# AlexFuster/Neural_network_image_compression

Hardware: AMD Instinct MI355X
Metric: Megapixels/sec encode+decode (higher is better)
Workload: dtype fp32 (split-f16x3 MFMA); 1 GPU; config2: 64x256x256x3 u8 synthetic per GPU, encode+decode (torch seed 1000+rank); global_batch=64, parallelism=dp1, weights=seeded spread init (random-init weights of the architecture)

## Files before the change

neural_network_image_compression_amd/csrc/nic_kernels.h:

```cpp
#pragma once
#include <hip/hip_runtime.h>
#include <stdint.h>

#include <vector>

namespace nic {

int set_error(int code, const char* msg);

enum InMode { IN_F32 = 0, IN_U8_LATENT = 1, IN_SPLIT = 2, IN_SPLIT_DMA = 3, IN_U8_CODES = 4 };
enum OutMode { OUT_F32 = 0, OUT_U8_LATENT = 1, OUT_SPLIT = 2 };

enum LayerId {
  L_CONV1 = 0, L_CONV2, L_CONV3, L_CONV4, L_CONV8,
  L_DCONV1, L_DCONV5, L_DCONV6, L_DCONV7, L_DCONV8,
  L_COUNT
};

constexpr float kF16Limit = 65504.0f;
struct RangeGuard {
  int* flag = nullptr;
  const int* gate = nullptr;
  int* trips = nullptr;
  int epoch = 0;
};

struct ConvArgs {
  RangeGuard rg;
  const float* in;
  const uint8_t* in_u8;
  float* out;
  const float* res;
  const uint16_t* in_s;
  uint16_t* out_s;
  const uint16_t* res_s;
  const char* zero16;
  uint8_t* out_u8;
  float* out_f32_latent;
  const float* w;
  const uint16_t* wx;
  float wscale[2];
  const float* bias;
  int P, nimg;
  int H, W;
  int OH, OW;
  int pad_y, pad_x;
  int tiles_x;
  int tiles_y, ntiles;
  int ws_taps;
  int ws_ngrp;
  int ws_blk[9];
  int ws_xcd;
  uint32_t* hist_part;
  const uint16_t* wx2;
  float wscale2[2];
  const float* bias2;
  int seg_rows;
  const uint8_t* rgb;
  const uint16_t* wx1;
  float wscale1[2];
  const float* bias1;
  int H0, W0;
  int p1y, p1x;
  uint16_t* cplane;
  int cp_h, cp_w;
  float* proj;
  const uint16_t* proj_w;
  float proj_scale[2];
};

struct Conv1Args {
  RangeGuard rg;
  const uint8_t* rgb;
  float* out;
  uint16_t* out_s;
// ... 159 lines not shown
```

neural_network_image_compression_amd/csrc/nic_kernels.hip:

```cpp

#include <hip/hip_runtime.h>
#include <stdint.h>
#include <stdlib.h>
#include <string.h>

#include <algorithm>
#include <type_traits>
#include <utility>

#include "nic_kernels.h"


namespace nic {

static int device_cus();

typedef float f32x2 __attribute__((ext_vector_type(2)));
typedef float f32x4 __attribute__((ext_vector_type(4)));
template <class F, int... I>
__device__ __forceinline__ void static_for_impl(F&& f, std::integer_sequence<int, I...>) {
  (f(std::integral_constant<int, I>{}), ...);
}
template <int N, class F>
__device__ __forceinline__ void static_for(F&& f) {
// ... 433 lines not shown
                                        int gx0, int c, int pw) const {
#pragma unroll
    for (int i = 0; i < NPP; ++i) {
      const int piece = pw + i * NPW;
      if (NPP * NPW > NPIECE && piece >= NPIECE) break;
      int e = code[i];
      if constexpr (OPAQUE) asm volatile("" : "+v"(e));
      const int gy = gy0 + (e & 255), gx = gx0 + ((e >> 8) & 255);
      const bool ok = (e >> 24) && (unsigned)gy < (unsigned)H && (unsigned)gx < (unsigned)W;
      const size_t off = ((size_t)(unsigned)(gy * W + gx) * CIN + (size_t)(((e >> 16) & 255) + c * HS) * 4) * 4;
      dma16(ok ? base + off : zero16, buf + piece * 1024);
    }
  }
};

constexpr unsigned kDmaOOR = 0x80000000u;
constexpr int kBufWord3 = 0x00020000;
#ifdef NIC_DIAG_KTIME
__device__ unsigned long long g_ktime[16][2];
#define KT_BEGIN(sl)                                                                         \
  do {                                                                                       \
    if ((threadIdx.x & 63) == 0) atomicMin(&g_ktime[sl][0], __builtin_amdgcn_s_memrealtime()); \
  } while (0)
#define KT_END(sl)                                                                           \
  do {                                                                                       \
    if ((threadIdx.x & 63) == 0) atomicMax(&g_ktime[sl][1], __builtin_amdgcn_s_memrealtime()); \
  } while (0)
struct KtGuard {
  int sl;
  __device__ explicit KtGuard(int s) : sl(s) { KT_BEGIN(s); }
  __device__ ~KtGuard() { KT_END(sl); }
};
#define KT_SCOPE(sl) KtGuard kt_guard_(sl)
extern "C" int nic_diag_ktime(unsigned long long* out, int reset) {
  if (out && hipMemcpyFromSymbol(out, HIP_SYMBOL(g_ktime), sizeof(g_ktime)) != hipSuccess) return -1;
  if (reset) {
    unsigned long long init[16][2];
    for (int k = 0; k < 16; ++k) init[k][0] = ~0ull, init[k][1] = 0;
    if (hipMemcpyToSymbol(HIP_SYMBOL(g_ktime), init, sizeof(init)) != hipSuccess) return -1;
  }
  return hipDeviceSynchronize() == hipSuccess ? 0 : -1;
}
#else
#define KT_BEGIN(sl) do { } while (0)
#define KT_END(sl) do { } while (0)
#define KT_SCOPE(sl) do { } while (0)
#endif

__device__ __forceinline__ void dma16_buf(__amdgpu_buffer_rsrc_t rsrc, unsigned voff, char* lds_wave_base) {
  __builtin_amdgcn_raw_ptr_buffer_load_lds(rsrc, (lds_ptr_t)lds_wave_base, 16, (int)voff, 0, 0, 0);
}

template <class G, int CIN, int NPW>
struct HaloDma {
  static_assert(G::HW <= 15, "halo column packed into the low 4 bits of a 16-B aligned offset");
  static constexpr int PSS = G::PSB / 16, RPS = G::RPB / 16;
  static constexpr int TOTAL = G::HH * RPS;
  static constexpr int NPIECE = (TOTAL + 63) / 64;
  static constexpr int NPP = (NPIECE + NPW - 1) / NPW;
  unsigned off[NPP];
  __device__ __forceinline__ void init(int pw, int lane, int W) {
#pragma unroll
// ... 90 lines not shown
    }
    pl += d_pl;
  }
};

template <int CIN, int TH, int TW>
struct GeomWS {
  static_assert(CIN == 64, "record geometry searched for Cin 64");
  static constexpr int HH = TH + 2, HW = TW + 2;
  static constexpr bool S2 = false, SWZ = true;
  static constexpr int HE = HW;
  static constexpr int PSB = CIN * 4;
  static constexpr int RPB = HW * PSB;
  static constexpr int HALO_BYTES = HH * RPB;
  static_assert(HALO_BYTES % 1024 == 0, "whole DMA pieces");
  static __device__ __forceinline__ int chunk_at(int slot, int hx) { return slot ^ ((2 * hx) & 15); }
};

#ifndef NIC_RES_DMA
#define NIC_RES_DMA 1
#endif
constexpr bool kResDma = NIC_RES_DMA != 0;
template <int CIN, int COUT, int TH, int TW, bool RESID, int KH, int KW, bool TRP, bool PROJ = false>
__device__ __forceinline__ void ws_body(const ConvArgs& a, char* lds, int model, int bi, int nb, int tb, int py,
                                        int px, bool copy_w8 = true) {
  constexpr int NTAPS = KH * KW, NW = COUT / 16, KST = CIN / 32, MT = TH * TW / 16;
  static_assert(TW == 8 && CIN % 32 == 0 && COUT % 16 == 0, "16-pixel tiles = two 8-pixel rows");
  static_assert(!(TRP && RESID), "no residual on the transposed phases");
  static_assert(!PROJ || (TRP && COUT == 64 && TH * TW == 64), "projection: dconv7 8x8 tiles");
  using G = GeomWS<CIN, TH, TW>;
  constexpr bool kBufHalo = !RESID || kResDma;
  using HP = std::conditional_t<kBufHalo, HaloDma<G, CIN, NW>, HaloPieces<G, CIN, CIN, NW>>;
  constexpr int TAP_BYTES = CIN * COUT * 4;

  const int wave = __builtin_amdgcn_readfirstlane(threadIdx.x >> 6);
  const int lane = threadIdx.x & 63, g = lane >> 4, l16 = lane & 15;
  const int co0 = wave * 16 + 4 * g;
  const int per_plane = a.tiles_y * a.tiles_x;
  const int p0 = model ? a.nimg : 0, np = model ? a.P - a.nimg : a.nimg;
  const int ntot = np * per_plane;
  const int ntile = bi < ntot ? (ntot - bi + nb - 1) / nb : 0;

  f16x8 wr[NTAPS][KST][2];
  {
    const char* wsrc = (const char*)a.wx + ((size_t)model * a.ws_taps + tb) * TAP_BYTES;
#pragma unroll
    for (int t = 0; t < NTAPS; ++t)
#pragma unroll
      for (int ks = 0; ks < KST; ++ks)
#pragma unroll
        for (int hl = 0; hl < 2; ++hl)
          wr[t][ks][hl] = *(const f16x8*)(wsrc + (size_t)t * TAP_BYTES +
                                          ((((2 * ks + (g >> 1)) * 2 + hl) * 2 + (g & 1)) * COUT + wave * 16 + l16) * 16);
  }
  const float scale = a.wscale[model];
  const f32x4 bias = *(const f32x4*)(a.bias + model * COUT + co0);
  constexpr int W8F = 2 * KST * 2;
  const f16x8* w8lds = (const f16x8*)(lds + 2 * G::HALO_BYTES) + lane;
  const float scale8 = PROJ ? a.proj_scale[model] : 0.f;
  char* hproj = lds + 2 * G::HALO_BYTES + W8F * 64 * 16;
  if constexpr (PROJ)
    if (copy_w8) {
      const f16x8* src = (const f16x8*)a.proj_w + (size_t)model * W8F * 64;
      for (int q = threadIdx.x; q < W8F * 64; q += 64 * NW) ((f16x8*)(lds + 2 * G::HALO_BYTES))[q] = src[q];
    }

  int bx[KW];
#pragma unroll
  for (int kw = 0; kw < KW; ++kw) {
    const int hx = (l16 & 7) + kw;
    bx[kw] = (l16 >> 3) * G::RPB + hx * G::PSB + (G::chunk_at(g, hx) << 4);
  }

  HP hp;
  const unsigned plane_bytes = (unsigned)((size_t)a.H * a.W * CIN * 4);
  if constexpr (kBufHalo)
    hp.init(wave, lane, a.W);
  else
    hp.init(wave, lane);
  TileWalk it_issue, it_ep;
  it_issue.init(bi, nb, a.tiles_y, a.tiles_x);
  it_ep = it_issue;
  auto tile_take = [&](TileWalk& w, int& p, int& t0y, int& t0x) {
    int pl, ty, tx;
    w.take(pl, ty, tx);
    p = p0 + pl;
    t0y = ty * TH;
    t0x = tx * TW;
  };
  auto issue = [&](int i) {
    int p, t0y, t0x;
    tile_take(it_issue, p, t0y, t0x);
#ifdef NIC_DIAG_ONETILE
    p = p0;
    t0y = TH;
    t0x = TW;
#endif
    if constexpr (kBufHalo)
      hp.issue(lds + (i & 1) * G::HALO_BYTES, (const char*)a.in_s + (size_t)p * plane_bytes, plane_bytes, a.W,
               t0y - a.pad_y, t0x - a.pad_x, wave);
    else
      hp.template issue<true>(lds + (i & 1) * G::HALO_BYTES, (const char*)a.in_s + (size_t)p * plane_bytes, a.zero16,
                              a.H, a.W, t0y - a.pad_y, t0x - a.pad_x, 0, wave);
  };
// ... 199 lines not shown
#endif
}

template <int CIN, int TH, int TW>
struct GeomS2 {
  static constexpr int HH = (TH - 1) * 2 + 5, HW = (TW - 1) * 2 + 5, HE = (HW + 1) / 2;
  static constexpr int PSS = CIN / 4 + 2, PSB = PSS * 16;
  static constexpr int RPS = (HW * PSS + 7) / 8 * 8, RPB = RPS * 16;
  static constexpr int HTOT = HH * RPS;
  static constexpr int NPIECE = (HTOT + 63) / 64;
  static constexpr int HALO_BYTES = NPIECE * 1024;
  static __device__ __forceinline__ int col(int hx) { return (hx & 1) * HE + (hx >> 1); }
};


constexpr int C12_PH = 41;

#ifndef NIC_WS2_PRIO
#define NIC_WS2_PRIO 1
#endif
constexpr int HIST_R = 2;
constexpr int HIST_LDS = 2 * 256 * HIST_R * 4 + 2 * 2 * 2 * 64 * 4;
template <int CIN, int COUT, int NTS, int TH, int OUT_MODE, int TS, bool HIST = false>
__device__ __forceinline__ void ws2_wave(const ConvArgs& a, char* lds, int model, int bi, int nb) {
  constexpr int TW = 8, MT = TH * TW / 16, NCG = COUT / 16, KST = CIN / 32, NW = NCG * NTS;
  static_assert(!HIST || OUT_MODE == OUT_U8_LATENT, "histogram fold: conv8 only");
  constexpr int T0 = 25 * TS / NTS, T1 = 25 * (TS + 1) / NTS, NT = T1 - T0;
  using G = GeomS2<CIN, TH, TW>;
  constexpr int TAP_BYTES = CIN * COUT * 4;
  constexpr int NPP = (G::NPIECE + NW - 1) / NW;
  constexpr int PART = MT * 1024;
  char* part = lds + 2 * G::HALO_BYTES;

  const int wave = __builtin_amdgcn_readfirstlane(threadIdx.x >> 6);
  const int cg = wave % NCG;
  const int lane = threadIdx.x & 63, g = lane >> 4, l16 = lane & 15;
  const int per_plane = a.tiles_y * a.tiles_x;
  const int p0 = model ? a.nimg : 0, np = model ? a.P - a.nimg : a.nimg;
  const int ntot = np * per_plane;
  const int ntile = bi < ntot ? (ntot - bi + nb - 1) / nb : 0;
  uint32_t* hist = (uint32_t*)(part + 2 * (NTS - 1) * NCG * PART);
  uint32_t* codes = hist + 2 * 256 * HIST_R;
  int hcur = 0, hpend = -1;
  uint32_t hz = 0;
  int h1_p = 0, h1_y = 0, h1_x = 0, h2_p = 0, h2_y = 0, h2_x = 0;
  auto hist_flush = [&](int q) __attribute__((always_inline)) {
    uint32_t* hb = hist + (q & 1) * (256 * HIST_R);
    const int t = cg * 64 + lane;
#pragma unroll
    for (int h = 0; h < 2; ++h) {
      const int bin = t + 128 * h;
      uint32_t c = 0;
#pragma unroll
      for (int r = 0; r < HIST_R; ++r) {
        c += hb[bin * HIST_R + r];
        hb[bin * HIST_R + r] = 0;
      }
      if (c) atomicAdd(a.hist_part + (size_t)(p0 + q) * 256 + bin, c);
    }
  };
  auto hist_close = [&] __attribute__((always_inline)) {
    uint32_t z = hz;
    for (int o = 32; o > 0; o >>= 1) z += __shfl_xor(z, o);
// ... 24 lines not shown
      }
    }
  };

  f16x8 wr[NT][KST][2];
  {
    const char* wsrc = (const char*)a.wx + ((size_t)model * 25 + T0) * TAP_BYTES;
#pragma unroll
    for (int t = 0; t < NT; ++t)
#pragma unroll
      for (int ks = 0; ks < KST; ++ks)
#pragma unroll
        for (int hl = 0; hl < 2; ++hl)
          wr[t][ks][hl] = *(const f16x8*)(wsrc + (size_t)t * TAP_BYTES +
                                          ((((2 * ks + (g >> 1)) * 2 + hl) * 2 + (g & 1)) * COUT + cg * 16 + l16) * 16);
  }
  const float scale = a.wscale[model];
  const int co0 = cg * 16 + 4 * g;
  const f32x4 bias = *(const f32x4*)(a.bias + model * COUT + co0);
  int boff[MT];
#pragma unroll
  for (int m = 0; m < MT; ++m) boff[m] = 2 * (2 * m + (l16 >> 3)) * G::RPB + (l16 & 7) * G::PSB + g * 16;
  TileWalk w_issue, w_ep;
  w_issue.init(bi, nb, a.tiles_y, a.tiles_x);
  w_ep = w_issue;
  if constexpr (HIST)
    for (int q = threadIdx.x; q < 2 * 256 * HIST_R; q += 64 * NW) hist[q] = 0;
  auto tile_take = [&](TileWalk& w, int& p, int& t0y, int& t0x) {
    int pl, ty, tx;
    w.take(pl, ty, tx);
    p = p0 + pl;
    t0y = ty * TH;
    t0x = tx * TW;
  };
  unsigned doff[NPP];
  int drc[NPP];
#pragma unroll
  for (int j = 0; j < NPP; ++j) {
    const int piece = wave + j * NW;
    const int q = piece * 64 + lane;
    const int row = q / G::RPS, r = q - row * G::RPS;
    const int sp = r / G::PSS, k = r - sp * G::PSS;
    const int hx = sp < G::HE ? 2 * sp : 2 * (sp - G::HE) + 1;
    const bool ok = piece < G::NPIECE && q < G::HTOT && sp < G::HW && k < CIN / 4;
    doff[j] = ok ? (unsigned)((row * a.W + hx) * CIN * 4 + k * 16) : kDmaOOR;
    drc[j] = row << 8 | hx;
  }
// ... 257 lines not shown
  }
#pragma unroll
  for (int k = 0; k < 3; ++k) {
    unsigned hw[2], lw[2];
#pragma unroll
    for (int h = 0; h < 2; ++h) {
      const _Float16 h0 = (_Float16)v[k][2 * h], h1 = (_Float16)v[k][2 * h + 1];
      const _Float16 l0 = (_Float16)(v[k][2 * h] - (float)h0), l1 = (_Float16)(v[k][2 * h + 1] - (float)h1);
      hw[h] = (unsigned)__builtin_bit_cast(uint16_t, h0) | (unsigned)__builtin_bit_cast(uint16_t, h1) << 16;
      lw[h] = (unsigned)__builtin_bit_cast(uint16_t, l0) | (unsigned)__builtin_bit_cast(uint16_t, l1) << 16;
    }
    const size_t o = ((size_t)k * N + n) * plane + (size_t)yp * wp + 4 * q4;
    typedef unsigned int u32x2v __attribute__((ext_vector_type(2)));
    __builtin_nontemporal_store((u32x2v){hw[0], hw[1]}, (u32x2v*)(cp + o));
    __builtin_nontemporal_store((u32x2v){lw[0], lw[1]}, (u32x2v*)(cp + P * plane + o));
  }
}


#ifndef NIC_C12_REUSE
#define NIC_C12_REUSE 1
#endif
template <int ROLE>
__device__ __forceinline__ void c12r_wave(const ConvArgs& a, char* lds, int model, int bi, int nb) {
  constexpr int CIN = 32, COUT = 64, MT = 4, NCG = 4;
  using G = GeomS2<CIN, 8, 8>;
  constexpr int TAP_BYTES = CIN * COUT * 4;
  constexpr int PART = MT * 1024;
  char* accs = lds + 2 * G::HALO_BYTES;
  char* patches = accs + NCG * PART;
  int* pflag = (int*)(patches + 4 * C12_PLANE);
  const int wave = __builtin_amdgcn_readfirstlane(threadIdx.x >> 6);
  const int cg = wave & 3;
  const int lane = threadIdx.x & 63, g = lane >> 4, l16 = lane & 15;
  const int per_plane = a.tiles_y * a.tiles_x;
  const int p0 = model ? a.nimg : 0, np = model ? a.P - a.nimg : a.nimg;
  const int ntot = np * per_plane;
  constexpr bool CONTIG = NIC_C12_REUSE != 0;
  const int t_first = CONTIG ? (int)((long long)bi * ntot / nb) : bi;
  const int ntile = CONTIG ? (int)((long long)(bi + 1) * ntot / nb) - t_first : bi < ntot ? (ntot - bi + nb - 1) / nb : 0;
  const int t_step = CONTIG ? 1 : nb;
  float rmax = 0.f;
  if (threadIdx.x < NCG) pflag[threadIdx.x] = 0;
#ifdef NIC_STAMPS
  unsigned long long sx[8] = {}, sa, sb;
  const unsigned long long s_rt0 = __builtin_amdgcn_s_memrealtime(), s_c0 = __builtin_amdgcn_s_memtime();
  NIC_PNOW(sa);
#define C12R_MARK(kk)  \
  do {                 \
    NIC_PNOW(sb);      \
    sx[kk] += sb - sa; \
    sa = sb;           \
  } while (0)
#else
#define C12R_MARK(kk) \
  do {                \
  } while (0)
#endif

  if constexpr (ROLE == 2) {
    f16x8 wr[25][2];
    {
      const char* wsrc = (const char*)a.wx + (size_t)model * 25 * TAP_BYTES;
#pragma unroll
// ... 228 lines not shown
    }
  }
#ifdef NIC_STAMPS
  if (lane == 0) {
    unsigned long long* o = g_stamps + ((size_t)blockIdx.x * 8 + wave) * 8;
#pragma unroll
    for (int q = 0; q < 7; ++q) o[q] = sx[q];
    o[7] = ntile;
    if (wave == 0) {
      g_stamps[256 * 64 + 2 * blockIdx.x] = __builtin_amdgcn_s_memtime() - s_c0;
      g_stamps[256 * 64 + 2 * blockIdx.x + 1] = __builtin_amdgcn_s_memrealtime() - s_rt0;
    }
  }
#endif
#undef C12R_MARK
  range_report(a.rg, rmax);
}

__device__ __forceinline__ int xcd_pos(int b, int nb) {
  const int x = b & 7, q = nb >> 3, r = nb & 7;
  return x * q + (x < r ? x : r) + (b >> 3);
}

__global__ __launch_bounds__(512) void conv12_kernel(ConvArgs a) {
  KT_SCOPE(1);
  using G = GeomS2<32, 8, 8>;
  __shared__ __attribute__((aligned(16)))
  char lds[2 * G::HALO_BYTES + 4 * 4 * 1024 + 4 * C12_PLANE + 16];
  int gi = 0;
  while (gi + 1 < a.ws_ngrp && (int)blockIdx.x >= a.ws_blk[gi + 1]) ++gi;
  const int nb = a.ws_blk[gi + 1] - a.ws_blk[gi];
  const int bi = xcd_pos(blockIdx.x - a.ws_blk[gi], nb);
  if (__builtin_amdgcn_readfirstlane((int)(threadIdx.x >> 6)) < 4)
    c12r_wave<2>(a, lds, gi, bi, nb);
  else
    c12r_wave<1>(a, lds, gi, bi, nb);
}

template <int CIN, int COUT, int NTS, int TH, int OUT_MODE, bool HIST = false>
__global__ __launch_bounds__(64 * (COUT / 16) * NTS) void conv_ws2_kernel(ConvArgs a) {
  KT_SCOPE(3);
  using G = GeomS2<CIN, TH, 8>;
  constexpr int NCG = COUT / 16;
  static_assert(NCG * NTS == 8, "8 waves per block");
  constexpr int PARTS = 2 * (NTS - 1) * NCG * (TH / 2) * 1024;
  __shared__ __attribute__((aligned(16)))
  char lds[2 * G::HALO_BYTES + PARTS + (HIST ? HIST_LDS : 0)];
  int gi = 0;
  while (gi + 1 < a.ws_ngrp && (int)blockIdx.x >= a.ws_blk[gi + 1]) ++gi;
  const int nb = a.ws_blk[gi + 1] - a.ws_blk[gi];
  const int bi = xcd_pos(blockIdx.x - a.ws_blk[gi], nb);
  const int ts = __builtin_amdgcn_readfirstlane((int)(threadIdx.x >> 6)) / NCG;
  static_for<NTS>([&](auto tsc) {
    constexpr int TS = decltype(tsc)::value;
    if (ts == TS) ws2_wave<CIN, COUT, NTS, TH, OUT_MODE, TS, HIST>(a, lds, gi, bi, nb);
  });
}

template <int CIN, int COUT, int TH, int TW, bool RESID, bool TRP, bool PROJ = false>
__global__ __launch_bounds__(64 * (COUT / 16), 2) void conv_ws_kernel(ConvArgs a) {
  KT_SCOPE(6);
  using G = GeomWS<CIN, TH, TW>;
  __shared__ __attribute__((aligned(16)))
  char lds[2 * G::HALO_BYTES + (PROJ ? 2 * (CIN / 32) * 2 * 64 * 16 + TH * TW * COUT * 4 : 0) +
           (RESID && kResDma ? (COUT / 16) * (TH * TW / 16) * 1024 : 0)];
  const int xcd = blockIdx.x & 7, ng = gridDim.x;
  const int lb = a.ws_xcd ? xcd * (ng >> 3) + min(xcd, ng & 7) + (int)(blockIdx.x >> 3) : (int)blockIdx.x;
  int gi = 0;
  while (gi + 1 < a.ws_ngrp && lb >= a.ws_blk[gi + 1]) ++gi;
  const int bi = lb - a.ws_blk[gi], nb = a.ws_blk[gi + 1] - a.ws_blk[gi];
  const int model = gi & 1;
  if constexpr (!TRP) {
    ws_body<CIN, COUT, TH, TW, RESID, 3, 3, false>(a, lds, model, bi, nb, 0, 0, 0);
  } else if (a.ws_ngrp == 2) {
    ws_body<CIN, COUT, TH, TW, false, 3, 3, true, PROJ>(a, lds, model, bi, nb, 16, 1, 1);
    ws_body<CIN, COUT, TH, TW, false, 2, 3, true, PROJ>(a, lds, model, bi, nb, 4, 0, 1, false);
    ws_body<CIN, COUT, TH, TW, false, 3, 2, true, PROJ>(a, lds, model, bi, nb, 10, 1, 0, false);
    ws_body<CIN, COUT, TH, TW, false, 2, 2, true, PROJ>(a, lds, model, bi, nb, 0, 0, 0, false);
  } else {
    switch (gi >> 1) {
      case 0: ws_body<CIN, COUT, TH, TW, false, 2, 2, true, PROJ>(a, lds, model, bi, nb, 0, 0, 0); break;
      case 1: ws_body<CIN, COUT, TH, TW, false, 2, 3, true, PROJ>(a, lds, model, bi, nb, 4, 0, 1); break;
      case 2: ws_body<CIN, COUT, TH, TW, false, 3, 2, true, PROJ>(a, lds, model, bi, nb, 10, 1, 0); break;
      default: ws_body<CIN, COUT, TH, TW, false, 3, 3, true, PROJ>(a, lds, model, bi, nb, 16, 1, 1); break;
    }
  }
}

constexpr int D1_PSB = 64;
constexpr int D1_RPB = 800;
constexpr int D1_HB = 10 * D1_RPB;
constexpr int D1A_LD = 2;
#ifndef NIC_D1A_PF
#define NIC_D1A_PF 2
#endif

template <int KH1, int KW1, int TB1, int PY1, int PX1, int KH2, int KW2, int TB2, int PY2, int PX2>
__device__ __forceinline__ void d1all_wave(const ConvArgs& a, char* lds, int model, int bi, int nb) {
  constexpr int COUT = 64, MT = 4, TAP_BYTES = 32 * COUT * 4, PXB = COUT * 4;
  constexpr int NT1 = KH1 * KW1, NT2 = KH2 * KW2;
  const int wave = __builtin_amdgcn_readfirstlane(threadIdx.x >> 6), cg = wave & 3;
  const int lane = threadIdx.x & 63, g = lane >> 4, l16 = lane & 15;
  const int per_plane = a.tiles_y * a.tiles_x;
  const int p0 = model ? a.nimg : 0, np = model ? a.P - a.nimg : a.nimg;
  const int ntot = np * per_plane;
  const int ntile = bi < ntot ? (ntot - bi + nb - 1) / nb : 0;
  if (ntile == 0) return;

  f16x8 w1[NT1][2], w2[NT2][2];
  float scale;
  f32x4 bias;
  auto load_weights = [&](int m) __attribute__((always_inline)) {
    const char* wsrc = (const char*)a.wx + (size_t)m * 25 * TAP_BYTES;
    auto frag_w = [&](int tap, int hl) {
      return *(const f16x8*)(wsrc + (size_t)tap * TAP_BYTES + ((((g >> 1) * 2 + hl) * 2 + (g & 1)) * COUT + cg * 16 + l16) * 16);
    };
#pragma unroll
    for (int t = 0; t < NT1; ++t)
#pragma unroll
      for (int hl = 0; hl < 2; ++hl) w1[t][hl] = frag_w(TB1 + t, hl);
#pragma unroll
    for (int t = 0; t < NT2; ++t)
#pragma unroll
      for (int hl = 0; hl < 2; ++hl) w2[t][hl] = frag_w(TB2 + t, hl);
    scale = a.wscale[m] * 0.0039215688593685627f;
    bias = *(const f32x4*)(a.bias + m * COUT + cg * 16 + 4 * g);
  };
  load_weights(model);

  int st_lds[D1A_LD], st_hy[D1A_LD], st_hx[D1A_LD];
#pragma unroll
  for (int j = 0; j < D1A_LD; ++j) {
    const int q = threadIdx.x + 512 * j, pix = q >> 3;
    st_hy[j] = q < 800 ? pix / 10 : -1000;
    st_hx[j] = pix - (pix / 10) * 10;
    st_lds[j] = (pix / 10) * D1_RPB + st_hx[j] * D1_PSB + (q & 7) * 8;
  }
  uint32_t cqa[D1A_LD], cqb[D1A_LD];
  TileWalk it_ld, it_run;
  it_ld.init(bi, nb, a.tiles_y, a.tiles_x);
  it_run = it_ld;
  const size_t img_bytes = (size_t)a.H * a.W * 96;
  auto load_codes = [&](uint32_t (&cq)[D1A_LD], bool live) __attribute__((always_inline)) {
    int pl, ty, tx;
    it_ld.take(pl, ty, tx);
    const int p = p0 + pl, type = p / a.nimg;
    const __amdgpu_buffer_rsrc_t rs = __builtin_amdgcn_make_buffer_rsrc(
        (void*)(a.in_u8 + (live ? (size_t)(p % a.nimg) * img_bytes + type * 32 : 0)), (short)0,
        live ? (int)(img_bytes - type * 32) : 0, kBufWord3);
#pragma unroll
    for (int j = 0; j < D1A_LD; ++j) {
      const int gy = ty * 8 - 1 + st_hy[j], gx = tx * 8 - 1 + st_hx[j];
      const bool ok = (unsigned)gy < (unsigned)a.H && (unsigned)gx < (unsigned)a.W;
      cq[j] = __builtin_amdgcn_raw_buffer_load_b32(
          rs, ok ? (unsigned)(((gy * a.W + gx) * 96) + (threadIdx.x & 7) * 4) : kDmaOOR, 0, 0);
    }
  };
  const int st_off = (g & 1) * COUT + cg * 16 + 8 * (g >> 1);
  const unsigned out_plane = (unsigned)((size_t)a.OH * a.OW * PXB);
  unsigned g_off[MT];
#pragma unroll
  for (int m = 0; m < MT; ++m) {
    const int dy = 2 * m + (l16 >> 3), dx = l16 & 7;
// ... 85 lines not shown
  load_codes(cqa, true);
  if constexpr (NIC_D1A_PF == 2) {
    load_codes(cqb, ntile > 1);
    {
      const __amdgpu_buffer_rsrc_t none = __builtin_amdgcn_make_buffer_rsrc((void*)a.out_s, (short)0, 0, kBufWord3);
#pragma unroll
      for (int k = 0; k < 16; ++k) __builtin_amdgcn_raw_buffer_store_b32(0u, none, kDmaOOR + 256u * k, 0, 0);
    }
    int i = 0;
    for (; i + 1 < ntile; i += 2) {
      step(i, cqa);
      step(i + 1, cqb);
    }
    if (i < ntile) step(i, cqa);
  } else {
    for (int i = 0; i < ntile; ++i) step(i, cqa);
  }
  range_report(a.rg, rmax);
}

__global__ __launch_bounds__(512, 1) void dconv1_all_kernel(ConvArgs a) {
  KT_SCOPE(5);
  __shared__ __attribute__((aligned(16))) char lds[2 * D1_HB];
  const int gi = (int)blockIdx.x >= a.ws_blk[1] ? 1 : 0;
  const int bi = blockIdx.x - a.ws_blk[gi], nb = a.ws_blk[gi + 1] - a.ws_blk[gi];
  if (threadIdx.x < 256)
    d1all_wave<3, 3, 16, 1, 1, 2, 2, 0, 0, 0>(a, lds, gi, bi, nb);
  else
    d1all_wave<2, 3, 4, 0, 1, 3, 2, 10, 1, 0>(a, lds, gi, bi, nb);
}

constexpr int K3P_MAX_W = 64;
constexpr int K3P_SW = 62;
constexpr int K3P_REC = 256;
constexpr int K3P_RW = K3P_MAX_W + 4;
constexpr int K3P_ROWB = K3P_RW * K3P_REC;
constexpr int K3P_NI = 5, K3P_NC = 4;
#ifndef NIC_K3P_DMAB
#define NIC_K3P_DMAB 1
#endif
constexpr bool kK3pDmaB = NIC_K3P_DMAB != 0;
constexpr int K3P_LDS = (K3P_NI + K3P_NC) * K3P_ROWB;

__device__ __forceinline__ int k3p_off(int rec, int chunk) { return rec * K3P_REC + ((chunk ^ ((2 * rec) & 15)) << 4); }

constexpr int K3P_MAX_GRID = 320;
struct K3Ranges {
  int start[K3P_MAX_GRID + 1];
};
template <int MT, bool SKEW, bool STRIP>
__global__ __launch_bounds__(512, 1) void conv_k3pair_kernel(ConvArgs a, K3Ranges rng) {
  KT_SCOPE(2);
// ... 943 lines not shown
static int device_cus() {
  static int cache[64] = {};
  int d = 0;
  if (hipGetDevice(&d) != hipSuccess || d < 0 || d >= 64) return 256;
  if (!cache[d]) {
    int n = 0;
    if (hipDeviceGetAttribute(&n, hipDeviceAttributeMultiprocessorCount, d) != hipSuccess || n <= 0) n = 256;
    cache[d] = n;
  }
  return cache[d];
}

template <int CIN, int COUT, int TH, int TW, bool RESID, bool TRP, bool PROJ = false>
static hipError_t launch_ws(ConvArgs a, hipStream_t st) {
  a.tiles_y = (a.H + TH - 1) / TH;
  a.tiles_x = (a.W + TW - 1) / TW;
  const long long per_plane = (long long)a.tiles_y * a.tiles_x;
  const long long nt = per_plane * a.P;
  if (nt == 0) return hipSuccess;
  if (nt > INT32_MAX || a.P != 3 * a.nimg) return hipErrorInvalidValue;
  if ((long long)a.H * a.W * CIN * 4 >= (1LL << 30)) return hipErrorInvalidValue;
  a.ntiles = (int)nt;
  a.ws_taps = TRP ? 25 : 9;
  a.ws_ngrp = 2;
  long long work[2], total = 0;
  for (int gi = 0; gi < 2; ++gi) {
    work[gi] = ((gi & 1) ? a.P - a.nimg : a.nimg) * per_plane;
    total += work[gi];
  }
  const int target = 2 * device_cus();
  a.ws_blk[0] = 0;
  for (int gi = 0; gi < a.ws_ngrp; ++gi) {
    const long long tiles = ((gi & 1) ? a.P - a.nimg : a.nimg) * per_plane;
    long long b = (work[gi] * target + total / 2) / total;
    b = b < 1 ? 1 : b > tiles ? tiles : b;
    a.ws_blk[gi + 1] = a.ws_blk[gi] + (int)b;
  }
  a.ws_xcd = 1;
  hipLaunchKernelGGL((conv_ws_kernel<CIN, COUT, TH, TW, RESID, TRP, PROJ>), dim3(a.ws_blk[a.ws_ngrp]),
                     dim3(64 * (COUT / 16)), 0, st, a);
  return hipGetLastError();
}

static void k3pair_balance(long long total, int H, int G, K3Ranges& r) {
  constexpr int F = 2;
  if (G <= 0 || G > K3P_MAX_GRID || total >= (1LL << 31) || H <= 0) return;
  auto fill = [&](long long T, bool write) {
    long long s = 0;
    int b = 0;
    while (s < total) {
      if (b == G) return G + 1;
      if (write) r.start[b] = (int)s;
      ++b;
      long long budget = T;
      while (s < total && budget > F) {
        const long long left = H - s % H, take = std::min(left, budget - F);
        s += take;
        budget -= take + F;
        if (take < left) break;
      }
    }
    if (write)
// ... 56 lines not shown
  if (nimg <= 0 || h8 <= 0 || w8 <= 0) return false;
  const long long pp = (long long)((h8 + 3) / 4) * ((w8 + 7) / 8);
  int by, bc;
  ws2_groups(nimg, pp, &by, &bc);
  return 2LL * by <= pp && 2LL * bc <= pp;
}

size_t hist_fold_scratch_bytes(int nimg, int h8, int w8) {
  (void)h8;
  (void)w8;
  return (size_t)3 * nimg * 256 * sizeof(uint32_t);
}

template <int CIN, int COUT, int NTS, int TH, int OUT_MODE, bool PIPE12 = false>
static hipError_t launch_ws2(ConvArgs a, hipStream_t st) {
  a.tiles_y = (a.OH + TH - 1) / TH;
  a.tiles_x = (a.OW + 7) / 8;
  const long long per_plane = (long long)a.tiles_y * a.tiles_x;
  const long long nt = per_plane * a.P;
  if (nt == 0) return hipSuccess;
  if (nt > INT32_MAX || a.P != 3 * a.nimg) return hipErrorInvalidValue;
  a.ntiles = (int)nt;
  a.ws_taps = 25;
  a.ws_ngrp = 2;
  int by, bc;
  ws2_groups(a.nimg, per_plane, &by, &bc);
  a.ws_blk[0] = 0;
  a.ws_blk[1] = by;
  a.ws_blk[2] = by + bc;
  if constexpr (PIPE12) {
    hipLaunchKernelGGL(conv12_kernel, dim3(a.ws_blk[2]), dim3(512), 0, st, a);
  } else if constexpr (OUT_MODE == OUT_U8_LATENT) {
    if (a.hist_part) {
      if (!hist_fold_supported(a.nimg, a.OH, a.OW)) return hipErrorInvalidValue;
      hipLaunchKernelGGL((conv_ws2_kernel<CIN, COUT, NTS, TH, OUT_MODE, true>), dim3(a.ws_blk[2]), dim3(512), 0, st, a);
    } else {
      hipLaunchKernelGGL((conv_ws2_kernel<CIN, COUT, NTS, TH, OUT_MODE>), dim3(a.ws_blk[2]), dim3(512), 0, st, a);
    }
  } else {
    hipLaunchKernelGGL((conv_ws2_kernel<CIN, COUT, NTS, TH, OUT_MODE>), dim3(a.ws_blk[2]), dim3(512), 0, st, a);
  }
  return hipGetLastError();
}

hipError_t launch_conv12_x3(const ConvArgs& a0, hipStream_t st) {
  ConvArgs a = a0;
  if (!a.rgb || !a.wx1 || !a.bias1 || a.H0 <= 0 || a.W0 <= 0) return hipErrorInvalidValue;
  if (!a.cplane || a.OH <= 0 || a.OW <= 0) return hipErrorInvalidValue;
  int oy, ox;
  c12_plane_geom(a.OH, a.OW, a.pad_y, a.pad_x, a.p1y, a.p1x, &oy, &ox, &a.cp_h, &a.cp_w);
  if ((long long)a.cp_h * a.cp_w * 2 >= (1LL << 31)) return hipErrorInvalidValue;
  const long long per_img = (long long)a.cp_h * (a.cp_w / 4);
  if (per_img == 0 || a.nimg == 0) return hipSuccess;
  if (a.nimg > 65535 || (long long)a.W0 * 3 >= (1LL << 31)) return hipErrorInvalidValue;
  hipLaunchKernelGGL(colour_split_kernel, dim3((unsigned)((per_img + 255) / 256), a.nimg),
                     dim3(256), 0, st, a.rgb, a.cplane, a.nimg, a.H0, a.W0, oy, ox, a.cp_h, a.cp_w);
  hipError_t e = hipGetLastError();
  if (e != hipSuccess) return e;
  return launch_ws2<32, 64, 2, 8, OUT_SPLIT, true>(a, st);
}

static hipError_t launch_dconv1_all(ConvArgs a, hipStream_t st) {
  a.tiles_y = (a.H + 7) / 8;
  a.tiles_x = (a.W + 7) / 8;
  const long long per_plane = (long long)a.tiles_y * a.tiles_x, nt = per_plane * a.P;
  if (nt == 0) return hipSuccess;
  if (nt > INT32_MAX || a.P != 3 * a.nimg || a.OH != 2 * a.H || a.OW != 2 * a.W || !a.in_u8) return hipErrorInvalidValue;
  if ((long long)a.OH * a.OW * 256 >= (1LL << 31)) return hipErrorInvalidValue;
  const long long target = device_cus();
  const long long ty = (long long)a.nimg * per_plane, tc = 2LL * a.nimg * per_plane;
  const int by = (int)std::max(1LL, std::min(ty, (target + 1) / 3)), bc = (int)std::max(1LL, std::min(tc, target - by));
  a.ws_ngrp = 2;
  a.ws_blk[0] = 0;
  a.ws_blk[1] = by;
  a.ws_blk[2] = by + bc;
  hipLaunchKernelGGL(dconv1_all_kernel, dim3(a.ws_blk[2]), dim3(512), 0, st, a);
  return hipGetLastError();
}

hipError_t launch_layer_x3(LayerId id, const ConvArgs& a, hipStream_t st) {
  switch (id) {
    case L_CONV2:
      return launch_ws2<32, 64, 2, 8, OUT_SPLIT>(a, st);
    case L_CONV3:
    case L_DCONV5:
      return launch_ws<64, 64, 8, 8, false, false>(a, st);
    case L_CONV4:
    case L_DCONV6:
      return launch_ws<64, 64, 8, 8, true, false>(a, st);
    case L_CONV8:
      return launch_ws2<64, 32, 4, 4, OUT_U8_LATENT>(a, st);
    case L_DCONV1:
      return launch_dconv1_all(a, st);
    default:
      return hipErrorInvalidValue;
// ... 94 lines not shown
```

Before: 3243 MP/s.

## Balance conv1/conv2 fused kernel with contiguous tile split across model boundary

Replaces the fixed per-model block grouping of the fused conv1+conv2 kernel with one global contiguous split of all tiles across a grid sized to the CU count. A block whose range straddles the luma/chroma boundary now runs two segments with a barrier between them. Other conv kernels are refactored onto a shared segment descriptor, which drops the multi-group search loop and the one-phase-per-block transposed path. The intent is to remove load imbalance and tail idle time, at the cost of an extra weight reload and barrier for straddling blocks. A per-block exit-time diagnostic is added behind a debug macro.

After: 3249 MP/s, median of 6. No clear change (+0.2%).

```diff
diff --git a/neural_network_image_compression_amd/csrc/nic_kernels.h b/neural_network_image_compression_amd/csrc/nic_kernels.h
--- a/neural_network_image_compression_amd/csrc/nic_kernels.h
+++ b/neural_network_image_compression_amd/csrc/nic_kernels.h
@@ -3,6 +3,8 @@
 #include <stdint.h>
 
 #include <vector>
+
+#include "nic_ws_split.h"
 
 namespace nic {
 
@@ -48,9 +50,8 @@
   int tiles_x;
   int tiles_y, ntiles;
   int ws_taps;
-  int ws_ngrp;
-  int ws_blk[9];
-  int ws_xcd;
+  WsSplit ws;
+  int ws_blk[3];
   uint32_t* hist_part;
   const uint16_t* wx2;
   float wscale2[2];
diff --git a/neural_network_image_compression_amd/csrc/nic_kernels.hip b/neural_network_image_compression_amd/csrc/nic_kernels.hip
--- a/neural_network_image_compression_amd/csrc/nic_kernels.hip
+++ b/neural_network_image_compression_amd/csrc/nic_kernels.hip
@@ -479,9 +479,15 @@
   do {                                                                                       \
     if ((threadIdx.x & 63) == 0) atomicMin(&g_ktime[sl][0], __builtin_amdgcn_s_memrealtime()); \
   } while (0)
+constexpr int kKtBlocks = 1024;
+__device__ unsigned long long g_kexit[16][kKtBlocks];
 #define KT_END(sl)                                                                           \
   do {                                                                                       \
-    if ((threadIdx.x & 63) == 0) atomicMax(&g_ktime[sl][1], __builtin_amdgcn_s_memrealtime()); \
+    if ((threadIdx.x & 63) == 0) {                                                           \
+      const unsigned long long kt_now_ = __builtin_amdgcn_s_memrealtime();                   \
+      atomicMax(&g_ktime[sl][1], kt_now_);                                                   \
+      atomicMax(&g_kexit[sl][blockIdx.x % kKtBlocks], kt_now_);                              \
+    }                                                                                        \
   } while (0)
 struct KtGuard {
   int sl;
@@ -495,6 +501,16 @@
     unsigned long long init[16][2];
     for (int k = 0; k < 16; ++k) init[k][0] = ~0ull, init[k][1] = 0;
     if (hipMemcpyToSymbol(HIP_SYMBOL(g_ktime), init, sizeof(init)) != hipSuccess) return -1;
+  }
+  return hipDeviceSynchronize() == hipSuccess ? 0 : -1;
+}
+extern "C" int nic_diag_kexit(int slot, unsigned long long* out, int reset) {
+  if (slot < 0 || slot >= 16) return -1;
+  const size_t off = (size_t)slot * kKtBlocks * sizeof(unsigned long long), n = kKtBlocks * sizeof(unsigned long long);
+  if (out && hipMemcpyFromSymbol(out, HIP_SYMBOL(g_kexit), n, off) != hipSuccess) return -1;
+  if (reset) {
+    void* p = nullptr;
+    if (hipGetSymbolAddress(&p, HIP_SYMBOL(g_kexit)) != hipSuccess || hipMemset((char*)p + off, 0, n) != hipSuccess) return -1;
   }
   return hipDeviceSynchronize() == hipSuccess ? 0 : -1;
 }
@@ -631,8 +647,8 @@
 #endif
 constexpr bool kResDma = NIC_RES_DMA != 0;
 template <int CIN, int COUT, int TH, int TW, bool RESID, int KH, int KW, bool TRP, bool PROJ = false>
-__device__ __forceinline__ void ws_body(const ConvArgs& a, char* lds, int model, int bi, int nb, int tb, int py,
-                                        int px, bool copy_w8 = true) {
+__device__ __forceinline__ void ws_body(const ConvArgs& a, char* lds, const WsSeg& sg, int tb, int py, int px,
+                                        bool copy_w8 = true) {
   constexpr int NTAPS = KH * KW, NW = COUT / 16, KST = CIN / 32, MT = TH * TW / 16;
   static_assert(TW == 8 && CIN % 32 == 0 && COUT % 16 == 0, "16-pixel tiles = two 8-pixel rows");
   static_assert(!(TRP && RESID), "no residual on the transposed phases");
@@ -645,10 +661,8 @@
   const int wave = __builtin_amdgcn_readfirstlane(threadIdx.x >> 6);
   const int lane = threadIdx.x & 63, g = lane >> 4, l16 = lane & 15;
   const int co0 = wave * 16 + 4 * g;
-  const int per_plane = a.tiles_y * a.tiles_x;
-  const int p0 = model ? a.nimg : 0, np = model ? a.P - a.nimg : a.nimg;
-  const int ntot = np * per_plane;
-  const int ntile = bi < ntot ? (ntot - bi + nb - 1) / nb : 0;
+  const int model = sg.model, ntile = sg.count;
+  const int p0 = model ? a.nimg : 0;
 
   f16x8 wr[NTAPS][KST][2];
   {
@@ -688,7 +702,7 @@
   else
     hp.init(wave, lane);
   TileWalk it_issue, it_ep;
-  it_issue.init(bi, nb, a.tiles_y, a.tiles_x);
+  it_issue.init(sg.first, sg.step, a.tiles_y, a.tiles_x);
   it_ep = it_issue;
   auto tile_take = [&](TileWalk& w, int& p, int& t0y, int& t0x) {
     int pl, ty, tx;
@@ -934,7 +948,7 @@
 constexpr int HIST_R = 2;
 constexpr int HIST_LDS = 2 * 256 * HIST_R * 4 + 2 * 2 * 2 * 64 * 4;
 template <int CIN, int COUT, int NTS, int TH, int OUT_MODE, int TS, bool HIST = false>
-__device__ __forceinline__ void ws2_wave(const ConvArgs& a, char* lds, int model, int bi, int nb) {
+__device__ __forceinline__ void ws2_wave(const ConvArgs& a, char* lds, const WsSeg& sg) {
   constexpr int TW = 8, MT = TH * TW / 16, NCG = COUT / 16, KST = CIN / 32, NW = NCG * NTS;
   static_assert(!HIST || OUT_MODE == OUT_U8_LATENT, "histogram fold: conv8 only");
   constexpr int T0 = 25 * TS / NTS, T1 = 25 * (TS + 1) / NTS, NT = T1 - T0;
@@ -947,10 +961,8 @@
   const int wave = __builtin_amdgcn_readfirstlane(threadIdx.x >> 6);
   const int cg = wave % NCG;
   const int lane = threadIdx.x & 63, g = lane >> 4, l16 = lane & 15;
-  const int per_plane = a.tiles_y * a.tiles_x;
-  const int p0 = model ? a.nimg : 0, np = model ? a.P - a.nimg : a.nimg;
-  const int ntot = np * per_plane;
-  const int ntile = bi < ntot ? (ntot - bi + nb - 1) / nb : 0;
+  const int model = sg.model, ntile = sg.count;
+  const int p0 = model ? a.nimg : 0;
   uint32_t* hist = (uint32_t*)(part + 2 * (NTS - 1) * NCG * PART);
   uint32_t* codes = hist + 2 * 256 * HIST_R;
   int hcur = 0, hpend = -1;
@@ -1021,7 +1033,7 @@
 #pragma unroll
   for (int m = 0; m < MT; ++m) boff[m] = 2 * (2 * m + (l16 >> 3)) * G::RPB + (l16 & 7) * G::PSB + g * 16;
   TileWalk w_issue, w_ep;
-  w_issue.init(bi, nb, a.tiles_y, a.tiles_x);
+  w_issue.init(sg.first, sg.step, a.tiles_y, a.tiles_x);
   w_ep = w_issue;
   if constexpr (HIST)
     for (int q = threadIdx.x; q < 2 * 256 * HIST_R; q += 64 * NW) hist[q] = 0;
@@ -1325,7 +1337,7 @@
 #define NIC_C12_REUSE 1
 #endif
 template <int ROLE>
-__device__ __forceinline__ void c12r_wave(const ConvArgs& a, char* lds, int model, int bi, int nb) {
+__device__ __forceinline__ void c12r_wave(const ConvArgs& a, char* lds, const WsSeg& sg) {
   constexpr int CIN = 32, COUT = 64, MT = 4, NCG = 4;
   using G = GeomS2<CIN, 8, 8>;
   constexpr int TAP_BYTES = CIN * COUT * 4;
@@ -1336,13 +1348,10 @@
   const int wave = __builtin_amdgcn_readfirstlane(threadIdx.x >> 6);
   const int cg = wave & 3;
   const int lane = threadIdx.x & 63, g = lane >> 4, l16 = lane & 15;
-  const int per_plane = a.tiles_y * a.tiles_x;
-  const int p0 = model ? a.nimg : 0, np = model ? a.P - a.nimg : a.nimg;
-  const int ntot = np * per_plane;
+  const int model = sg.model, ntile = sg.count;
+  const int p0 = model ? a.nimg : 0;
   constexpr bool CONTIG = NIC_C12_REUSE != 0;
-  const int t_first = CONTIG ? (int)((long long)bi * ntot / nb) : bi;
-  const int ntile = CONTIG ? (int)((long long)(bi + 1) * ntot / nb) - t_first : bi < ntot ? (ntot - bi + nb - 1) / nb : 0;
-  const int t_step = CONTIG ? 1 : nb;
+  const int t_first = sg.first, t_step = sg.step;
   float rmax = 0.f;
   if (threadIdx.x < NCG) pflag[threadIdx.x] = 0;
 #ifdef NIC_STAMPS
@@ -1617,19 +1626,36 @@
   return x * q + (x < r ? x : r) + (b >> 3);
 }
 
+__device__ __forceinline__ WsSeg group_seg(const ConvArgs& a, int b, bool xcd) {
+  const int gi = b >= a.ws_blk[1] ? 1 : 0;
+  const int nb = a.ws_blk[gi + 1] - a.ws_blk[gi], bi = xcd ? xcd_pos(b - a.ws_blk[gi], nb) : b - a.ws_blk[gi];
+  const int ntot = (gi ? a.P - a.nimg : a.nimg) * a.tiles_y * a.tiles_x;
+  return WsSeg{gi, bi, nb, bi < ntot ? (ntot - bi + nb - 1) / nb : 0};
+}
+
+__device__ __forceinline__ WsSeg seg_uniform(const WsSeg& g) {
+  return WsSeg{__builtin_amdgcn_readfirstlane(g.model), __builtin_amdgcn_readfirstlane(g.first),
+               __builtin_amdgcn_readfirstlane(g.step), __builtin_amdgcn_readfirstlane(g.count)};
+}
+
 __global__ __launch_bounds__(512) void conv12_kernel(ConvArgs a) {
   KT_SCOPE(1);
   using G = GeomS2<32, 8, 8>;
   __shared__ __attribute__((aligned(16)))
   char lds[2 * G::HALO_BYTES + 4 * 4 * 1024 + 4 * C12_PLANE + 16];
-  int gi = 0;
-  while (gi + 1 < a.ws_ngrp && (int)blockIdx.x >= a.ws_blk[gi + 1]) ++gi;
-  const int nb = a.ws_blk[gi + 1] - a.ws_blk[gi];
-  const int bi = xcd_pos(blockIdx.x - a.ws_blk[gi], nb);
-  if (__builtin_amdgcn_readfirstlane((int)(threadIdx.x >> 6)) < 4)
-    c12r_wave<2>(a, lds, gi, bi, nb);
-  else
-    c12r_wave<1>(a, lds, gi, bi, nb);
+  WsSeg s0, s1;
+  const int nseg = ws_split_segs(a.ws, xcd_pos(blockIdx.x, gridDim.x), s0, s1);
+  auto run = [&](const WsSeg& sg) __attribute__((always_inline)) {
+    if (__builtin_amdgcn_readfirstlane((int)(threadIdx.x >> 6)) < 4)
+      c12r_wave<2>(a, lds, sg);
+    else
+      c12r_wave<1>(a, lds, sg);
+  };
+  run(seg_uniform(s0));
+  if (nseg == 2) {
+    __syncthreads();
+    run(seg_uniform(s1));
+  }
 }
 
 template <int CIN, int COUT, int NTS, int TH, int OUT_MODE, bool HIST = false>
@@ -1641,14 +1667,11 @@
   constexpr int PARTS = 2 * (NTS - 1) * NCG * (TH / 2) * 1024;
   __shared__ __attribute__((aligned(16)))
   char lds[2 * G::HALO_BYTES + PARTS + (HIST ? HIST_LDS : 0)];
-  int gi = 0;
-  while (gi + 1 < a.ws_ngrp && (int)blockIdx.x >= a.ws_blk[gi + 1]) ++gi;
-  const int nb = a.ws_blk[gi + 1] - a.ws_blk[gi];
-  const int bi = xcd_pos(blockIdx.x - a.ws_blk[gi], nb);
+  const WsSeg sg = group_seg(a, blockIdx.x, true);
   const int ts = __builtin_amdgcn_readfirstlane((int)(threadIdx.x >> 6)) / NCG;
   static_for<NTS>([&](auto tsc) {
     constexpr int TS = decltype(tsc)::value;
-    if (ts == TS) ws2_wave<CIN, COUT, NTS, TH, OUT_MODE, TS, HIST>(a, lds, gi, bi, nb);
+    if (ts == TS) ws2_wave<CIN, COUT, NTS, TH, OUT_MODE, TS, HIST>(a, lds, sg);
   });
 }
 
@@ -1659,26 +1682,14 @@
   __shared__ __attribute__((aligned(16)))
   char lds[2 * G::HALO_BYTES + (PROJ ? 2 * (CIN / 32) * 2 * 64 * 16 + TH * TW * COUT * 4 : 0) +
            (RESID && kResDma ? (COUT / 16) * (TH * TW / 16) * 1024 : 0)];
-  const int xcd = blockIdx.x & 7, ng = gridDim.x;
-  const int lb = a.ws_xcd ? xcd * (ng >> 3) + min(xcd, ng & 7) + (int)(blockIdx.x >> 3) : (int)blockIdx.x;
-  int gi = 0;
-  while (gi + 1 < a.ws_ngrp && lb >= a.ws_blk[gi + 1]) ++gi;
-  const int bi = lb - a.ws_blk[gi], nb = a.ws_blk[gi + 1] - a.ws_blk[gi];
-  const int model = gi & 1;
+  const WsSeg sg = group_seg(a, xcd_pos(blockIdx.x, gridDim.x), false);
   if constexpr (!TRP) {
-    ws_body<CIN, COUT, TH, TW, RESID, 3, 3, false>(a, lds, model, bi, nb, 0, 0, 0);
-  } else if (a.ws_ngrp == 2) {
-    ws_body<CIN, COUT, TH, TW, false, 3, 3, true, PROJ>(a, lds, model, bi, nb, 16, 1, 1);
-    ws_body<CIN, COUT, TH, TW, false, 2, 3, true, PROJ>(a, lds, model, bi, nb, 4, 0, 1, false);
-    ws_body<CIN, COUT, TH, TW, false, 3, 2, true, PROJ>(a, lds, model, bi, nb, 10, 1, 0, false);
-    ws_body<CIN, COUT, TH, TW, false, 2, 2, true, PROJ>(a, lds, model, bi, nb, 0, 0, 0, false);
+    ws_body<CIN, COUT, TH, TW, RESID, 3, 3, false>(a, lds, sg, 0, 0, 0);
   } else {
-    switch (gi >> 1) {
-      case 0: ws_body<CIN, COUT, TH, TW, false, 2, 2, true, PROJ>(a, lds, model, bi, nb, 0, 0, 0); break;
-      case 1: ws_body<CIN, COUT, TH, TW, false, 2, 3, true, PROJ>(a, lds, model, bi, nb, 4, 0, 1); break;
-      case 2: ws_body<CIN, COUT, TH, TW, false, 3, 2, true, PROJ>(a, lds, model, bi, nb, 10, 1, 0); break;
-      default: ws_body<CIN, COUT, TH, TW, false, 3, 3, true, PROJ>(a, lds, model, bi, nb, 16, 1, 1); break;
-    }
+    ws_body<CIN, COUT, TH, TW, false, 3, 3, true, PROJ>(a, lds, sg, 16, 1, 1);
+    ws_body<CIN, COUT, TH, TW, false, 2, 3, true, PROJ>(a, lds, sg, 4, 0, 1, false);
+    ws_body<CIN, COUT, TH, TW, false, 3, 2, true, PROJ>(a, lds, sg, 10, 1, 0, false);
+    ws_body<CIN, COUT, TH, TW, false, 2, 2, true, PROJ>(a, lds, sg, 0, 0, 0, false);
   }
 }
 
@@ -1691,15 +1702,13 @@
 #endif
 
 template <int KH1, int KW1, int TB1, int PY1, int PX1, int KH2, int KW2, int TB2, int PY2, int PX2>
-__device__ __forceinline__ void d1all_wave(const ConvArgs& a, char* lds, int model, int bi, int nb) {
+__device__ __forceinline__ void d1all_wave(const ConvArgs& a, char* lds, const WsSeg& sg) {
   constexpr int COUT = 64, MT = 4, TAP_BYTES = 32 * COUT * 4, PXB = COUT * 4;
   constexpr int NT1 = KH1 * KW1, NT2 = KH2 * KW2;
   const int wave = __builtin_amdgcn_readfirstlane(threadIdx.x >> 6), cg = wave & 3;
   const int lane = threadIdx.x & 63, g = lane >> 4, l16 = lane & 15;
-  const int per_plane = a.tiles_y * a.tiles_x;
-  const int p0 = model ? a.nimg : 0, np = model ? a.P - a.nimg : a.nimg;
-  const int ntot = np * per_plane;
-  const int ntile = bi < ntot ? (ntot - bi + nb - 1) / nb : 0;
+  const int model = sg.model, ntile = sg.count;
+  const int p0 = model ? a.nimg : 0;
   if (ntile == 0) return;
 
   f16x8 w1[NT1][2], w2[NT2][2];
@@ -1733,7 +1742,7 @@
   }
   uint32_t cqa[D1A_LD], cqb[D1A_LD];
   TileWalk it_ld, it_run;
-  it_ld.init(bi, nb, a.tiles_y, a.tiles_x);
+  it_ld.init(sg.first, sg.step, a.tiles_y, a.tiles_x);
   it_run = it_ld;
   const size_t img_bytes = (size_t)a.H * a.W * 96;
   auto load_codes = [&](uint32_t (&cq)[D1A_LD], bool live) __attribute__((always_inline)) {
@@ -1865,12 +1874,11 @@
 __global__ __launch_bounds__(512, 1) void dconv1_all_kernel(ConvArgs a) {
   KT_SCOPE(5);
   __shared__ __attribute__((aligned(16))) char lds[2 * D1_HB];
-  const int gi = (int)blockIdx.x >= a.ws_blk[1] ? 1 : 0;
-  const int bi = blockIdx.x - a.ws_blk[gi], nb = a.ws_blk[gi + 1] - a.ws_blk[gi];
+  const WsSeg sg = group_seg(a, blockIdx.x, false);
   if (threadIdx.x < 256)
-    d1all_wave<3, 3, 16, 1, 1, 2, 2, 0, 0, 0>(a, lds, gi, bi, nb);
+    d1all_wave<3, 3, 16, 1, 1, 2, 2, 0, 0, 0>(a, lds, sg);
   else
-    d1all_wave<2, 3, 4, 0, 1, 3, 2, 10, 1, 0>(a, lds, gi, bi, nb);
+    d1all_wave<2, 3, 4, 0, 1, 3, 2, 10, 1, 0>(a, lds, sg);
 }
 
 constexpr int K3P_MAX_W = 64;
@@ -2860,22 +2868,15 @@
   if ((long long)a.H * a.W * CIN * 4 >= (1LL << 30)) return hipErrorInvalidValue;
   a.ntiles = (int)nt;
   a.ws_taps = TRP ? 25 : 9;
-  a.ws_ngrp = 2;
-  long long work[2], total = 0;
-  for (int gi = 0; gi < 2; ++gi) {
-    work[gi] = ((gi & 1) ? a.P - a.nimg : a.nimg) * per_plane;
-    total += work[gi];
-  }
+  const long long tiles[2] = {a.nimg * per_plane, (a.P - a.nimg) * per_plane};
   const int target = 2 * device_cus();
   a.ws_blk[0] = 0;
-  for (int gi = 0; gi < a.ws_ngrp; ++gi) {
-    const long long tiles = ((gi & 1) ? a.P - a.nimg : a.nimg) * per_plane;
-    long long b = (work[gi] * target + total / 2) / total;
-    b = b < 1 ? 1 : b > tiles ? tiles : b;
+  for (int gi = 0; gi < 2; ++gi) {
+    long long b = (tiles[gi] * target + nt / 2) / nt;
+    b = b < 1 ? 1 : b > tiles[gi] ? tiles[gi] : b;
     a.ws_blk[gi + 1] = a.ws_blk[gi] + (int)b;
   }
-  a.ws_xcd = 1;
-  hipLaunchKernelGGL((conv_ws_kernel<CIN, COUT, TH, TW, RESID, TRP, PROJ>), dim3(a.ws_blk[a.ws_ngrp]),
+  hipLaunchKernelGGL((conv_ws_kernel<CIN, COUT, TH, TW, RESID, TRP, PROJ>), dim3(a.ws_blk[2]),
                      dim3(64 * (COUT / 16)), 0, st, a);
   return hipGetLastError();
 }
@@ -2978,15 +2979,17 @@
   if (nt > INT32_MAX || a.P != 3 * a.nimg) return hipErrorInvalidValue;
   a.ntiles = (int)nt;
   a.ws_taps = 25;
-  a.ws_ngrp = 2;
+  if constexpr (PIPE12) {
+    if (!ws_split_plan(a.nimg * per_plane, 2 * a.nimg * per_plane, device_cus(), &a.ws)) return hipErrorInvalidValue;
+    hipLaunchKernelGGL(conv12_kernel, dim3(a.ws.grid), dim3(512), 0, st, a);
+    return hipGetLastError();
+  }
   int by, bc;
   ws2_groups(a.nimg, per_plane, &by, &bc);
   a.ws_blk[0] = 0;
   a.ws_blk[1] = by;
   a.ws_blk[2] = by + bc;
-  if constexpr (PIPE12) {
-    hipLaunchKernelGGL(conv12_kernel, dim3(a.ws_blk[2]), dim3(512), 0, st, a);
-  } else if constexpr (OUT_MODE == OUT_U8_LATENT) {
+  if constexpr (OUT_MODE == OUT_U8_LATENT) {
     if (a.hist_part) {
       if (!hist_fold_supported(a.nimg, a.OH, a.OW)) return hipErrorInvalidValue;
       hipLaunchKernelGGL((conv_ws2_kernel<CIN, COUT, NTS, TH, OUT_MODE, true>), dim3(a.ws_blk[2]), dim3(512), 0, st, a);
@@ -3026,7 +3029,6 @@
   const long long target = device_cus();
   const long long ty = (long long)a.nimg * per_plane, tc = 2LL * a.nimg * per_plane;
   const int by = (int)std::max(1LL, std::min(ty, (target + 1) / 3)), bc = (int)std::max(1LL, std::min(tc, target - by));
-  a.ws_ngrp = 2;
   a.ws_blk[0] = 0;
   a.ws_blk[1] = by;
   a.ws_blk[2] = by + bc;
diff --git a/neural_network_image_compression_amd/csrc/nic_ws_split.h b/neural_network_image_compression_amd/csrc/nic_ws_split.h
--- /dev/null
+++ b/neural_network_image_compression_amd/csrc/nic_ws_split.h
@@ -0,0 +1,50 @@
+#pragma once
+
+#if defined(__HIPCC__) || defined(__CUDACC__)
+#define NIC_HD __host__ __device__
+#else
+#define NIC_HD
+#endif
+
+namespace nic {
+
+struct WsSplit {
+  int grid;
+  int ty, tc;
+  int q, r;
+};
+
+struct WsSeg {
+  int model, first, step, count;
+};
+
+NIC_HD inline long long ws_split_start(const WsSplit& s, int b) { return (long long)b * s.q + (b < s.r ? b : s.r); }
+
+inline bool ws_split_plan(long long ty, long long tc, int target, WsSplit* s) {
+  const long long total = ty + tc;
+  if (ty <= 0 || tc <= 0 || target <= 0 || total > 0x7fffffffLL) return false;
+  s->grid = (int)(total < target ? total : target);
+  s->ty = (int)ty;
+  s->tc = (int)tc;
+  s->q = (int)(total / s->grid);
+  s->r = (int)(total % s->grid);
+  return true;
+}
+
+NIC_HD inline int ws_split_segs(const WsSplit& s, int b, WsSeg& s0, WsSeg& s1) {
+  const int g0 = (int)ws_split_start(s, b), g1 = (int)ws_split_start(s, b + 1);
+  s1 = WsSeg{1, 0, 1, 0};
+  if (g1 <= s.ty) {
+    s0 = WsSeg{0, g0, 1, g1 - g0};
+    return 1;
+  }
+  if (g0 >= s.ty) {
+    s0 = WsSeg{1, g0 - s.ty, 1, g1 - g0};
+    return 1;
+  }
+  s0 = WsSeg{0, g0, 1, s.ty - g0};
+  s1 = WsSeg{1, 0, 1, g1 - s.ty};
+  return 2;
+}
+
+}
```
